# rostin79s/TFHE-AES

Measured on AMD Instinct MI355X. Metric: AES-128 CTR blocks/sec (FHE), higher is better.
Workload: dtype u64+f64; 1 GPU; configs[2]: 128 CTR blocks per GPU, Server::aes_encrypt 10 rounds (1280 bit-CBS/block), counters pre-incremented client-side; params=PARAM_OPT, blocks_per_gpu=128, total_blocks=128

## Files before the change

### include/fheaes.h

```cpp
#ifndef FHEAES_H
#define FHEAES_H

#include <stddef.h>
#include <stdint.h>

#ifdef __cplusplus
extern "C" {
#endif

#define FHEAES_OK 0
#define FHEAES_ERR_INVALID -1
#define FHEAES_ERR_NOKEYS -2
#define FHEAES_ERR_DEVICE -3
#define FHEAES_ERR_NOMEM -4

#define FHEAES_HOST 0
#define FHEAES_DEVICE 1

typedef struct fheaes_params {
    uint32_t lwe_dimension;
    uint32_t glwe_dimension;
    uint32_t polynomial_size;
    uint32_t pbs_base_log;
    uint32_t pbs_level;
// ... 215 lines not shown
int fheaes_profile_reset(fheaes_ctx *ctx);
int fheaes_profile_read(fheaes_ctx *ctx, int stage, double *total_ms, uint64_t *launches, uint64_t *units);

int fheaes_get_twiddles(double *psi_out);
int fheaes_read_bsk_fourier(fheaes_ctx *ctx, uint32_t i, double *out);
int fheaes_k2_launch_plan(uint64_t m, uint32_t cu_count, uint32_t k, int *form, uint64_t *units_main, uint32_t *r_main,
                          uint64_t *units_tail, uint32_t *r_tail);
int fheaes_k2_launch_plan_forms(uint64_t m, uint32_t cu_count, uint32_t k, int allow_pair, int *form, uint64_t *units_main, uint32_t *r_main,
                                uint64_t *units_tail, uint32_t *r_tail);
int fheaes_k2_context_plan(fheaes_ctx *ctx, uint64_t m, int *form, uint64_t *units_main, uint32_t *r_main, uint64_t *units_tail,
                           uint32_t *r_tail, char *kernel, size_t kernel_cap);
int fheaes_k2_set_parking(fheaes_ctx *ctx, int claimed);
int fheaes_k2_set_forms(fheaes_ctx *ctx, int allow_pair, int allow_home);
int fheaes_aes_window_plan(uint64_t n_blocks, uint32_t steps, uint32_t cu_count, uint32_t k, uint64_t *window_blocks, uint64_t *launches,
                           uint64_t *generations, uint64_t *generations_by_round);
int fheaes_aes_context_window(fheaes_ctx *ctx, uint64_t n_blocks, uint32_t steps, uint64_t *window_blocks);
#define FHEAES_AES_WINDOW_OFF 0xFFFFFFFFu
int fheaes_aes_set_window(fheaes_ctx *ctx, uint32_t window_blocks);
#define FHEAES_K2_PARK_SLOTS 1024
int fheaes_k2_park_debug(fheaes_ctx *ctx, const uint32_t *initial_owner, int record);
int fheaes_k2_park_read(fheaes_ctx *ctx, uint64_t *fallbacks, uint64_t *violations, uint32_t *owner_out, uint32_t *record_out,
                        uint64_t record_cap, uint64_t *record_n);
#define FHEAES_WS_BUFFERS 17
#define FHEAES_WS_F64 0
#define FHEAES_WS_WORDS 1
#define FHEAES_WS_TABLES 2
#define FHEAES_WS_PATTERN_F64_HALF 0x7FF87FF8u
#define FHEAES_WS_PATTERN_WORDS 0xA5
#define FHEAES_WS_PATTERN_TABLES 1u
#define FHEAES_WS_POISON_FILL 0
// ... 12 lines not shown
```

### tfhe_aes_amd/_native.py

```python
from __future__ import annotations

import ctypes
import os
import re
from pathlib import Path

import numpy as np

from . import _build
from .params import CParams, WopbsParameters

HOST, DEVICE = 0, 1
MAC_NONE = 0xFFFFFFFF
KW_MIN_SEMIBLOCKS, KW_MAX_SEMIBLOCKS, KW_MAX_KEYS = 2, 8, 4096
AES_WINDOW_OFF = 0xFFFFFFFF
GATE_LWE, GATE_GLWE = 0, 1
K2_PARK_SLOTS = 1024
AUDIT_MAX_ROWS, AUDIT_RECORDS = 256, 16
WS_BUFFERS = 17
WS_CLASSES = ("f64", "words", "tables")
WS_POISON_FILL, WS_POISON_RELEASE = 0, 1
STAGES = ("keyswitch", "blind_rotate", "pfpks", "ggsw_fft", "vertical_packing", "linear")

_u64p = ctypes.POINTER(ctypes.c_uint64)
# ... 111 lines not shown
    "fheaes_gate_plan": (_c.c_int, [_u64p, _c.c_uint64, _c.c_uint32, _u64p, _u32p]),
    "fheaes_profile_enable": (_c.c_int, [_ctx, _c.c_int]),
    "fheaes_profile_reset": (_c.c_int, [_ctx]),
    "fheaes_profile_read": (_c.c_int, [_ctx, _c.c_int, _dp, _u64p, _u64p]),
    "fheaes_get_twiddles": (_c.c_int, [_dp]),
    "fheaes_read_bsk_fourier": (_c.c_int, [_ctx, _c.c_uint32, _dp]),
    "fheaes_k2_launch_plan": (_c.c_int, [_c.c_uint64, _c.c_uint32, _c.c_uint32, _c.POINTER(_c.c_int), _c.POINTER(_c.c_uint64), _c.POINTER(_c.c_uint32),
                                       _c.POINTER(_c.c_uint64), _c.POINTER(_c.c_uint32)]),
    "fheaes_k2_launch_plan_forms": (_c.c_int, [_c.c_uint64, _c.c_uint32, _c.c_uint32, _c.c_int, _c.POINTER(_c.c_int), _c.POINTER(_c.c_uint64),
                                             _c.POINTER(_c.c_uint32), _c.POINTER(_c.c_uint64), _c.POINTER(_c.c_uint32)]),
    "fheaes_k2_context_plan": (_c.c_int, [_ctx, _c.c_uint64, _c.POINTER(_c.c_int), _c.POINTER(_c.c_uint64), _c.POINTER(_c.c_uint32),
                                        _c.POINTER(_c.c_uint64), _c.POINTER(_c.c_uint32), _c.c_char_p, _c.c_size_t]),
    "fheaes_k2_set_parking": (_c.c_int, [_ctx, _c.c_int]),
    "fheaes_k2_set_forms": (_c.c_int, [_ctx, _c.c_int, _c.c_int]),
    "fheaes_aes_window_plan": (_c.c_int, [_c.c_uint64, _c.c_uint32, _c.c_uint32, _c.c_uint32, _u64p, _u64p, _u64p, _u64p]),
    "fheaes_aes_context_window": (_c.c_int, [_ctx, _c.c_uint64, _c.c_uint32, _u64p]),
    "fheaes_aes_set_window": (_c.c_int, [_ctx, _c.c_uint32]),
    "fheaes_k2_park_debug": (_c.c_int, [_ctx, _c.POINTER(_c.c_uint32), _c.c_int]),
    "fheaes_k2_park_read": (_c.c_int, [_ctx, _u64p, _u64p, _c.POINTER(_c.c_uint32), _c.POINTER(_c.c_uint32), _c.c_uint64, _u64p]),
    "fheaes_audit_set": (_c.c_int, [_ctx, _c.c_uint32, _c.c_uint64, _c.c_uint64]),
    "fheaes_audit_rows": (_c.c_int, [_c.c_uint64, _c.c_uint64, _c.c_uint64, _c.c_uint32, _u64p]),
    "fheaes_audit_read": (_c.c_int, [_ctx, _u64p, _u64p, _u64p, _u64p, _c.c_uint64, _u64p]),
    "fheaes_audit_debug": (_c.c_int, [_ctx, _c.c_uint64, _c.c_uint32, _c.c_uint64]),
    "fheaes_workspace_info": (_c.c_int, [_ctx, _c.c_uint32, _c.c_char_p, _c.c_size_t, _u64p, _c.POINTER(_c.c_int), _u64p, _u64p]),
    "fheaes_workspace_poison": (_c.c_int, [_ctx, _c.c_int, _u64p]),
    "fheaes_alloc_debug": (_c.c_int, [_ctx, _c.c_uint64, _u64p]),
    "fheaes_version": (_c.c_char_p, []),
}

_libs = {}
# ... 658 lines not shown
    out = np.zeros(14, dtype=np.uint64)
    rc = load_library().fheaes_aes_public_plan(cnt.ctypes.data_as(_u64p), len(cnt), key_bits, out.ctypes.data_as(_u64p))
    if rc != 0:
        raise FheAesError(rc, "fheaes_aes_public_plan: key_bits must be 128, 192 or 256")
    return [int(x) for x in out[:{128: 10, 192: 12, 256: 14}[key_bits]]]


def aes_window_plan(n_blocks: int, steps: int, cu_count: int = 256, k: int = 4) -> dict:
    w, la, g, gr = _c.c_uint64(), _c.c_uint64(), _c.c_uint64(), _c.c_uint64()
    rc = load_library().fheaes_aes_window_plan(n_blocks, steps, cu_count, k, _c.byref(w), _c.byref(la), _c.byref(g), _c.byref(gr))
    if rc != 0:
        raise FheAesError(rc, "fheaes_aes_window_plan: n_blocks, steps and cu_count must be at least 1")
    return {"window": w.value, "launches": la.value, "generations": g.value, "generations_by_round": gr.value}


def get_twiddles() -> np.ndarray:
    out = np.empty((512, 2), dtype=np.float64)
    rc = load_library().fheaes_get_twiddles(out.ctypes.data_as(_dp))
    if rc != 0:
        raise FheAesError(rc, "fheaes_get_twiddles")
    return out


def gen_lut(nb_block: int, f_table) -> np.ndarray:
    f = np.ascontiguousarray(f_table, dtype=np.uint64)
    if f.size != 1 << nb_block:
        raise ValueError("f_table must have 2^nb_block entries")
    out = np.empty((nb_block, max(512, 1 << nb_block)), dtype=np.uint64)
    rc = load_library().fheaes_gen_lut(nb_block, f.ctypes.data_as(_u64p), out.ctypes.data_as(_u64p))
    if rc != 0:
# ... 3 lines not shown
```

### tfhe_aes_amd/csrc/aes_schedule.h

```cpp
#pragma once

static int many_sbox_dev(fheaes_ctx *c, const uint64_t *bytes, uint64_t n_bytes, int set, uint64_t *out)
{
    return wopbs_dev(c, bytes, n_bytes, 8, c->lutset_d[set], (uint32_t)c->lutset_n[set], 0, out);
}

static int aes_rounds(uint32_t key_bits) { return key_bits == 128 ? 10 : key_bits == 192 ? 12 : key_bits == 256 ? 14 : 0; }

static int check_key_bits(fheaes_ctx *c, uint32_t key_bits)
{
    if (!aes_rounds(key_bits)) return c->fail(FHEAES_ERR_INVALID, "key_bits must be 128, 192 or 256, got %u", key_bits);
    return FHEAES_OK;
}

struct AesStep { int set; uint32_t n_luts; GatherTable table; int key_round; };
struct AesSchedule {
    int first_key_round = 0;
    uint32_t max_luts = 0;
    std::vector<AesStep> steps;
    void add(int set, uint32_t n_luts, const GatherTable &t, int key_round) { steps.push_back({set, n_luts, t, key_round}); max_luts = std::max(max_luts, n_luts); }
};

static AesSchedule aes_encrypt_schedule(int nr)
{
// ... 31 lines not shown
    auto key_of = [&](const AesStep &st, uint64_t first_block) {
        if (st.key_round < 0) return KeySets{nullptr, nullptr, 0};
        return rk.round((uint64_t)st.key_round, sw, first_block);
    };
    const uint64_t w = aes_context_window(c, n_blocks, steps);
    TRY(ensure(c, c->ws_vp, (w ? w : n_blocks) * 16 * sch.max_luts * bw * 8));
    uint64_t *vp = (uint64_t *)c->ws_vp.p;
    TRY(launch_add_bcast(c, state, rk.round((uint64_t)sch.first_key_round, sw), sw, n_blocks));
    if (w == 0) {
        for (const AesStep &st : sch.steps) {
            TRY(many_sbox_dev(c, state, 16 * n_blocks, st.set, vp));
            TRY(launch_gather(c, vp, st.n_luts, key_of(st, 0), state, n_blocks, st.table));
        }
        return FHEAES_OK;
    }
    const uint64_t ggsw_words = (uint64_t)c->k1 * c->k1 * FHE_N, total = steps * n_blocks;
    TRY(ensure_wopbs_ws(c, w * AES_BLOCK_BITS));
    uint64_t *small = (uint64_t *)c->ws_small.p;
    const double2 *ggswf = (const double2 *)c->ws_ggswf.p;
    struct Segment { const AesStep *st; uint64_t first, blocks, row; uint64_t *vp; };
    for (uint64_t i0 = 0; i0 < total; i0 += w) {
        const uint64_t len = std::min<uint64_t>(w, total - i0), s = i0 / n_blocks, b0 = i0 % n_blocks, m = len * AES_BLOCK_BITS;
        Segment seg[2] = {{&sch.steps[s], b0, std::min<uint64_t>(len, n_blocks - b0), 0, vp}, {}};
        int n_seg = 1;
        if (seg[0].blocks < len) {
            seg[1] = {&sch.steps[s + 1], 0, len - seg[0].blocks, seg[0].blocks, vp + seg[0].blocks * 16 * seg[0].st->n_luts * bw};
            n_seg = 2;
        }
        for (int g = 0; g < n_seg; ++g)
            TRY(launch_keyswitch(c, state + seg[g].first * sw, seg[g].blocks * AES_BLOCK_BITS, small + seg[g].row * AES_BLOCK_BITS * (c->n + 1)));
        TRY(cbs_from_small(c, m));
        if (n_seg == 1 || seg[0].st->set == seg[1].st->set) {
            const int set = seg[0].st->set;
            TRY(launch_vertical_packing(c, ggswf, 16 * len, 8, c->lutset_d[set], (uint32_t)c->lutset_n[set], 0, vp));
        } else {
            for (int g = 0; g < n_seg; ++g) {
                const int set = seg[g].st->set;
                TRY(launch_vertical_packing(c, ggswf + seg[g].row * AES_BLOCK_BITS * (ggsw_words / 2), 16 * seg[g].blocks, 8, c->lutset_d[set],
                                            (uint32_t)c->lutset_n[set], 0, seg[g].vp));
            }
        }
        for (int g = 0; g < n_seg; ++g)
            TRY(launch_gather(c, seg[g].vp, seg[g].st->n_luts, key_of(*seg[g].st, seg[g].first), state + seg[g].first * sw, seg[g].blocks, seg[g].st->table));
    }
    return FHEAES_OK;
}

static int aes_encrypt_dev(fheaes_ctx *c, const KeySets &rk, uint64_t *state, uint64_t n_blocks, int nr) { return aes_run_dev(c, rk, state, n_blocks, aes_encrypt_schedule(nr)); }
static int aes_decrypt_dev(fheaes_ctx *c, const KeySets &rk, uint64_t *state, uint64_t n_blocks, int nr) { return aes_run_dev(c, rk, state, n_blocks, aes_decrypt_schedule(nr)); }
static int aes_decrypt_eq_dev(fheaes_ctx *c, const KeySets &dw, uint64_t *state, uint64_t n_blocks, int nr) { return aes_run_dev(c, dw, state, n_blocks, aes_decrypt_eq_schedule(nr)); }

typedef int (*AesDevFn)(fheaes_ctx *, const KeySets &, uint64_t *, uint64_t, int);

static int dec_round_keys_dev(fheaes_ctx *c, const uint64_t *w, uint64_t *dw, int nr, uint64_t n_keys)
// ... 500 lines not shown
```

### tfhe_aes_amd/csrc/engine.hip

```cpp
#include <hip/hip_runtime.h>
#include <algorithm>
#include <cmath>
#include <cstdarg>
#include <cstdio>
#include <atomic>
#include <chrono>
#include <cstring>
#include <functional>
#include <mutex>
#include <string>
#include <type_traits>
#include <unordered_map>
#include <vector>

#include "knobs.h"
#include "fheaes.h"
#include "fft_dev.h"
#include "kern_extprod.h"
#include "kern_gate.h"
#include "kern_blindrot_latency.h"
#include "kern_blindrot16.h"
#include "kern_blindrot_pair.h"
#include "kern_audit.h"
#include "ks_launch.h"
// ... 69 lines not shown
    if (!ctx) return FHEAES_ERR_INVALID;
    CtxLock lock__(ctx);
    if ((allow_pair != 0 && allow_pair != 1) || (allow_home != 0 && allow_home != 1))
        return ctx->fail(FHEAES_ERR_INVALID, "k2_set_forms: each of allow_pair, allow_home is 0 or 1 (got %d, %d)", allow_pair, allow_home);
    HIP_TRY(ctx, hipStreamSynchronize(ctx->stream));
    ctx->k2_deny_pair = allow_pair == 0;
    ctx->k2_deny_home = allow_home == 0;
    return FHEAES_OK;
}
int fheaes_aes_window_plan(uint64_t n_blocks, uint32_t steps, uint32_t cu_count, uint32_t k, uint64_t *window_blocks, uint64_t *launches,
                           uint64_t *generations, uint64_t *generations_by_round)
{
    if (!window_blocks || !launches || !generations || !generations_by_round || n_blocks == 0 || steps == 0 || cu_count == 0) return FHEAES_ERR_INVALID;
    const AesWindowPlan pl = aes_window_plan(n_blocks, steps, cu_count, k + 1);
    *window_blocks = pl.window; *launches = pl.launches; *generations = pl.generations; *generations_by_round = pl.generations_by_round;
    return FHEAES_OK;
}
int fheaes_aes_context_window(fheaes_ctx *ctx, uint64_t n_blocks, uint32_t steps, uint64_t *window_blocks)
{
    if (!ctx) return FHEAES_ERR_INVALID;
    CtxLock lock__(ctx);
    if (!window_blocks) return ctx->fail(FHEAES_ERR_INVALID, "aes_context_window: null output");
    *window_blocks = aes_context_window(ctx, n_blocks, steps);
    return FHEAES_OK;
}
int fheaes_aes_set_window(fheaes_ctx *ctx, uint32_t window_blocks)
{
    if (!ctx) return FHEAES_ERR_INVALID;
    CtxLock lock__(ctx);
    HIP_TRY(ctx, hipStreamSynchronize(ctx->stream));
// ... 1872 lines not shown
```

### tfhe_aes_amd/csrc/engine_launch.h

```cpp
#pragma once

#define MAX_CHUNK_BITS 32768ull
#define K2_CALL_MAX_BITS 65536ull
#define MAX_WOPBS_BITS 16u

namespace {

#define LATENCY_BATCH_BITS 256ull
#define K2_PAIR_MIN_BITS 768ull
struct K2Plan { int form; uint64_t units_main; uint32_t r_main; uint64_t units_tail; uint32_t r_tail; };
K2Plan k2_plan(uint64_t m, uint32_t cu_count, uint32_t k1, bool allow_pair = true)
{
    K2Plan pl{};
    if (m <= LATENCY_BATCH_BITS) { pl.form = 0; pl.units_main = m; pl.r_main = 1; return pl; }
    if (allow_pair && k1 == 5 && m > K2_PAIR_MIN_BITS) {
        pl.form = 2; pl.r_main = 6; pl.r_tail = 4;
        const uint64_t gens = (m + 6ull * cu_count - 1) / (6ull * cu_count);
        uint64_t nu = gens * cu_count;
        uint64_t four = 6 * nu >= m ? (6 * nu - m) / 2 : 0;
        if (four > nu) four = nu;
        if (four == nu && 4 * nu > m) { nu = (m + 3) / 4; four = nu; }
        pl.units_tail = four; pl.units_main = nu - four;
        return pl;
    }
// ... 47 lines not shown
    const uint64_t gen_bits = 6ull * cu_count;
    if (k2_plan(std::min<uint64_t>(n * AES_BLOCK_BITS, MAX_CHUNK_BITS), cu_count, k1, allow_pair).form != 2) return pl;
    if (n * AES_BLOCK_BITS % gen_bits == 0) return pl;
    uint64_t g = AES_BLOCK_BITS, r = gen_bits;
    while (r) { const uint64_t t = g % r; g = r; r = t; }
    const uint64_t base = gen_bits / g;
    const uint64_t w = std::min<uint64_t>(n, AES_WINDOW_MAX_BLOCKS) / base * base;
    if (w == 0) return pl;
    uint64_t launches, generations;
    aes_window_count(n, steps, w, cu_count, k1, &launches, &generations);
    if (generations >= pl.generations_by_round) return pl;
    pl.window = w; pl.launches = launches; pl.generations = generations;
    return pl;
}

int launch_keyswitch(fheaes_ctx *c, const uint64_t *in, uint64_t m, uint64_t *out)
{
    if (m == 0) return FHEAES_OK;
    StageScope sc(c, FHEAES_STAGE_KEYSWITCH, m);
    const uint64_t ct_tiles16 = ((m + KS_CT_TILE - 1) / KS_CT_TILE) * (KS_CT_TILE / 16);
    TRY(ensure(c, c->ws_digits, ct_tiles16 * c->ks_ksteps * 1024));
    int8_t *af = (int8_t *)c->ws_digits.p;
    const uint64_t threads = ct_tiles16 * c->ks_ksteps * 64;
    ks_launch_digits_k1(dim3((unsigned)((threads + 255) / 256)), c->stream, in, (uint64_t)c->big1, c->big, m, c->ks_ksteps, af);
    KeyswitchArgs a{};
    a.afrag = af; a.bfrag = c->ksk_frag; a.ksteps = c->ks_ksteps; a.coltiles = c->ks_coltiles;
    a.in = in; a.in_stride = c->big1; a.body_index = (int32_t)c->big; a.body_col = c->n; a.ncols = c->n + 1;
    a.out = out; a.out_stride = c->n + 1; a.out_z_stride = 0; a.m = m;
    dim3 grid((c->ks_coltiles + KSL_COL_TILES - 1) / KSL_COL_TILES, (unsigned)((m + 16 * KSL_CT_TILES - 1) / (16 * KSL_CT_TILES)), 1);
    ks_launch_mfma_lds(1, grid, c->stream, a);
    HIP_TRY(c, hipGetLastError());
    return FHEAES_OK;
}

int launch_pfpks(fheaes_ctx *c, const uint64_t *in, uint64_t m, uint64_t *out, uint64_t out_stride, int block = -1)
{
    if (m == 0) return FHEAES_OK;
    StageScope sc(c, FHEAES_STAGE_PFPKS, m);
    const uint32_t gsz = c->k1 * FHE_N;
    const uint64_t ct_tiles16 = ((m + KS_CT_TILE - 1) / KS_CT_TILE) * (KS_CT_TILE / 16);
    TRY(ensure(c, c->ws_digits, ct_tiles16 * c->pf_ksteps * 2 * 1024));
    int8_t *af = (int8_t *)c->ws_digits.p;
    const uint64_t threads = ct_tiles16 * c->pf_ksteps * 64;
    ks_launch_digits_k3(dim3((unsigned)((threads + 255) / 256)), c->stream, in, (uint64_t)c->big1, c->big1, m, c->pf_ksteps, af);
    KeyswitchArgs a{};
    a.afrag = af; a.bfrag = c->pfpksk_frag; a.ksteps = c->pf_ksteps; a.coltiles = c->pf_coltiles;
    if (block >= 0) a.bfrag += (size_t)block * c->pf_ksteps * c->pf_coltiles * 8 * 1024;
    a.in = in; a.in_stride = c->big1; a.body_index = -1; a.body_col = 0; a.ncols = gsz;
    a.out = out; a.out_stride = out_stride; a.out_z_stride = block >= 0 ? 0 : gsz; a.m = m;
    dim3 grid((c->pf_coltiles + KSL_COL_TILES - 1) / KSL_COL_TILES, (unsigned)((m + 16 * KSL_CT_TILES - 1) / (16 * KSL_CT_TILES)), block >= 0 ? 1 : c->k1);
    ks_launch_mfma_lds(2, grid, c->stream, a);
    HIP_TRY(c, hipGetLastError());
    return FHEAES_OK;
}

int launch_forward_fourier(fheaes_ctx *c, const uint64_t *in, uint64_t polys, double2 *out, int stage)
{
    if (polys == 0) return FHEAES_OK;
    StageScope sc(c, stage, polys);
    uint64_t wgs = (polys + EP_GROUPS - 1) / EP_GROUPS;
    if (wgs > 8192) wgs = 8192;
    hipLaunchKernelGGL(forward_fourier_kernel, dim3((unsigned)wgs), dim3(EP_THREADS), 0, c->stream, in, out, polys, c->tw_d);
    HIP_TRY(c, hipGetLastError());
    return FHEAES_OK;
}

bool k2_pair_allowed(fheaes_ctx *c)
{
    if (c->k2_deny_pair) return false;
    if (c->k2_pair_ok < 0) {
        int per_cu = 0;
        const hipError_t oe = hipOccupancyMaxActiveBlocksPerMultiprocessor(&per_cu, blind_rotate_pair_kernel<5, 5, 8, 3, 2>, BRP_THREADS, 0);
        c->k2_pair_ok = (oe == hipSuccess && per_cu >= 1) ? 1 : 0;
        (void)hipGetLastError();
    }
    return c->k2_pair_ok == 1;
}
// ... 131 lines not shown
#ifdef EP_STAMPS
    static const char *namesL[EP_NPH] = {"barrier (result) + accumulate", "rotate+decompose (1 coeff x K1)", "read digits + forward fft", "digit stores", "barrier (digits)", "MAC", "barrier (MAC done)",
                                         "products store + next rows", "barrier (products)", "inverse fft -> doubles", "barrier (acc)", "barrier (decomposition)"};
    static const char *namesT[EP_NPH] = {"stage+rotate+decomp_first", "decomp_next", "fwd head", "pre-level barrier", "fwd tail (transpose+dft16)",
                                         "digit stores+late loads", "exchange barrier", "MAC", "products exchange", "inverse fft", "convert+add", "loop head"};
    StampReport rep(c, (size_t)L.grid * (L.threads / 64), L.pl.form == 0 ? namesL : namesT, L.pl.form == 0 ? 8 : 0);
    a.stamps = rep.d;
#endif
    hipLaunchKernelGGL(L.kernel, dim3(L.grid), dim3(L.threads), 0, c->stream, a);
    HIP_TRY(c, hipGetLastError());
    if (c->audit_rows && m >= c->audit_min_bits) TRY(launch_audit(c, a));
    return FHEAES_OK;
}

int launch_vertical_packing(fheaes_ctx *c, const double2 *ggswf, uint64_t n_inputs, uint32_t bits, const uint64_t *luts,
                            uint32_t n_luts, int per_input, uint64_t *out)
{
    if (n_inputs == 0) return FHEAES_OK;
    StageScope sc(c, FHEAES_STAGE_VERTICAL_PACKING, n_inputs * n_luts * bits);
    const bool k4 = c->k1 == 5;
    const uint32_t R = k4 ? 3 : 8;
    void (*const cmux_kernel)(CmuxArgs) = k4 ? cmux_level_kernel<5, 15, 3> : cmux_level_kernel<2, 15, 8>;
    void (*const vp_kernel)(VpArgs) = k4 ? vertical_packing_kernel<5, 15, 3> : vertical_packing_kernel<2, 15, 8>;
    const uint32_t inst_per_input = n_luts * bits;
    const uint64_t W = lut_row_words(bits);
    const uint64_t *glwe_root = nullptr;
    if (bits > 9) {
        const uint32_t tree_bits = bits - 9;
        const uint64_t instances = n_inputs * inst_per_input, gsz = (uint64_t)c->k1 * FHE_N;
        const uint64_t half_words = instances * (1ull << (tree_bits - 1)) * gsz;
        TRY(ensure(c, c->ws_tree, 2 * half_words * 8));
        uint64_t *buf[2] = {(uint64_t *)c->ws_tree.p, (uint64_t *)c->ws_tree.p + half_words};
        for (uint32_t t = 0; t < tree_bits; ++t) {
            CmuxArgs a{};
            a.ggsw = ggswf; a.tw = c->tw_d;
            a.luts = t == 0 ? luts : nullptr; a.in = t == 0 ? nullptr : buf[(t - 1) & 1]; a.out = buf[t & 1];
            a.bits = bits; a.bit = 9 + t; a.nodes_out = 1u << (tree_bits - 1 - t);
            a.inst_per_input = inst_per_input; a.lut_per_input = per_input ? 1 : 0; a.lut_words = W;
            const uint64_t jobs = (uint64_t)inst_per_input * a.nodes_out;
            a.wg_per_input = (uint32_t)((jobs + R - 1) / R);
            hipLaunchKernelGGL(cmux_kernel, dim3((unsigned)(n_inputs * a.wg_per_input)), dim3(EP_THREADS), 0, c->stream, a);
            HIP_TRY(c, hipGetLastError());
        }
        glwe_root = buf[(tree_bits - 1) & 1];
    }
    VpArgs a{};
    a.ggsw = ggswf; a.tw = c->tw_d;
    a.out = out; a.iters = bits < 9 ? bits : 9; a.ggsw_per_input = bits;
    a.luts = luts; a.lut_words = W; a.glwe_in = glwe_root;
    a.lut_per_input = per_input ? 1 : 0; a.inst_per_input = inst_per_input;
    a.wg_per_input = (inst_per_input + R - 1) / R;
    hipLaunchKernelGGL(vp_kernel, dim3((unsigned)(n_inputs * a.wg_per_input)), dim3(EP_THREADS), 0, c->stream, a);
    HIP_TRY(c, hipGetLastError());
    return FHEAES_OK;
}

#define GATE_MAX_GRID 65536ull
uint32_t gate_r(uint32_t k1) { return k1 == 5 ? 3 : 8; }

uint64_t gate_table(const uint64_t *bits_of_gate, uint64_t n_gates, uint32_t R, uint64_t chunk, std::vector<GateWg> *wgs, std::vector<uint64_t> *chunk_end,
                    uint64_t *n_wgs)
{
    uint64_t first = 0, count = 0;
// ... 285 lines not shown
    if (!c) return FHEAES_ERR_INVALID;
    if (!c->have_keys) return c->fail(FHEAES_ERR_NOKEYS, "evaluation keys have not been uploaded");
    return FHEAES_OK;
}

int ensure_wopbs_ws(fheaes_ctx *c, uint64_t bits)
{
    const uint64_t ggsw_words = (uint64_t)c->k1 * c->k1 * FHE_N;
    TRY(ensure(c, c->ws_small, bits * (c->n + 1) * 8));
    TRY(ensure(c, c->ws_pbs, bits * c->big1 * 8));
    TRY(ensure(c, c->ws_ggsw, bits * ggsw_words * 8));
    TRY(ensure(c, c->ws_ggswf, bits * ggsw_words * 8));
    return FHEAES_OK;
}

int cbs_from_small(fheaes_ctx *c, uint64_t m)
{
    const uint64_t ggsw_words = (uint64_t)c->k1 * c->k1 * FHE_N;
    TRY(launch_cbs_pbs(c, (const uint64_t *)c->ws_small.p, m, 1, (uint64_t *)c->ws_pbs.p));
    TRY(launch_pfpks(c, (const uint64_t *)c->ws_pbs.p, m, (uint64_t *)c->ws_ggsw.p, ggsw_words));
    TRY(launch_forward_fourier(c, (const uint64_t *)c->ws_ggsw.p, m * c->k1 * c->k1, (double2 *)c->ws_ggswf.p, FHEAES_STAGE_GGSW_FFT));
    return FHEAES_OK;
}

int cbs_bits(fheaes_ctx *c, const uint64_t *in, uint64_t m)
{
    TRY(launch_keyswitch(c, in, m, (uint64_t *)c->ws_small.p));
    return cbs_from_small(c, m);
}

int wopbs_dev(fheaes_ctx *c, const uint64_t *lwe_in, uint64_t n_inputs, uint32_t bits, const uint64_t *luts, uint32_t n_luts,
              int per_input, uint64_t *lwe_out)
{
    if (bits < 1 || bits > MAX_WOPBS_BITS) return c->fail(FHEAES_ERR_INVALID, "bits_per_input must be in 1..%u (got %u)", MAX_WOPBS_BITS, bits);
    if (n_luts < 1) return c->fail(FHEAES_ERR_INVALID, "n_luts must be >= 1");
    if (n_inputs == 0) return FHEAES_OK;
    uint64_t chunk_inputs = std::max<uint64_t>(1, MAX_CHUNK_BITS / bits);
    if (bits > 9) {
        const uint64_t per_input = (uint64_t)n_luts * bits * (1ull << (bits - 9)) * c->k1 * FHE_N * 8;
        chunk_inputs = std::max<uint64_t>(1, std::min<uint64_t>(chunk_inputs, (2ull << 30) / per_input));
    }
    const uint64_t W = lut_row_words(bits);
    TRY(ensure_wopbs_ws(c, std::min<uint64_t>(n_inputs, chunk_inputs) * bits));
    for (uint64_t i0 = 0; i0 < n_inputs; i0 += chunk_inputs) {
        const uint64_t ni = std::min<uint64_t>(chunk_inputs, n_inputs - i0);
        TRY(cbs_bits(c, lwe_in + i0 * bits * c->big1, ni * bits));
        const uint64_t *l = per_input ? luts + i0 * n_luts * bits * W : luts;
        TRY(launch_vertical_packing(c, (const double2 *)c->ws_ggswf.p, ni, bits, l, n_luts, per_input, lwe_out + i0 * n_luts * bits * c->big1));
    }
    return FHEAES_OK;
}

}
```

### tfhe_aes_amd/csrc/kern_extprod.h

```cpp
#pragma once
#include "fft_dev.h"

#define EP_THREADS 256
#define EP_EARLY_LOAD 2
#define EP_MAC_PRIO 1
#define EP_ROT_CHUNK 4
#define EP_PREFETCH 2
#define EP_MIN_WAVES 2
#define EP_GROUPS 16
#define EP_LDS_DOUBLES (EP_GROUPS * GROUP_TILE_DOUBLES + 2 * FHE_TW_ENTRIES)

__device__ __forceinline__ void ep_load_table(double2 *tw_lds, const double2 *tw_g)
{
    for (int i = threadIdx.x; i < FHE_TW_ENTRIES; i += blockDim.x) tw_lds[i] = tw_g[i];
}

struct ExtProdArgs {
    const double2 *ggsw;
    const double2 *tw;
    uint64_t *out;
    uint64_t count;
    uint32_t iters;
    const uint64_t *lwe_in;
    uint64_t tv_const;
// ... 67 lines not shown
        double2 v = *reinterpret_cast<const double2 *>(tile + 2 * (b + 16 * k2));
        xr[k2] = v.x; xi[k2] = v.y;
    }
    wave_lds_sync();
    nega_inv(xr, xi, tw, tile, b);
}

#ifdef EP_STAMPS
#define EP_NPH 12
#define EP_STAMP(ph) do { unsigned long long t__ = __builtin_readcyclecounter(); ph_cyc[ph] += t__ - t_last; t_last = t__; } while (0)
#else
#define EP_STAMP(ph) do { } while (0)
#endif

struct VpArgs {
    const double2 *ggsw;
    const double2 *tw;
    uint64_t *out;
    uint32_t iters;
    const uint64_t *luts;
    uint32_t lut_per_input;
    uint32_t inst_per_input;
    uint32_t wg_per_input;
    uint32_t ggsw_per_input;
    uint64_t lut_words;
    const uint64_t *glwe_in;
};

template <int K1, int BASE_LOG, int R>
__global__ __launch_bounds__(EP_THREADS, EP_MIN_WAVES) void vertical_packing_kernel(const VpArgs A)
{
    static_assert(R * K1 <= EP_GROUPS, "too many polynomials for 16 lane groups");
    __shared__ __attribute__((aligned(16))) double lds[EP_LDS_DOUBLES];
    double2 *tw = reinterpret_cast<double2 *>(lds + EP_GROUPS * GROUP_TILE_DOUBLES);

    const int tid = threadIdx.x;
    const int g = tid >> 4, b = tid & 15;
    const bool owner = g < R * K1;
    const int r_own = owner ? g / K1 : R - 1;
// ... 14 lines not shown
#pragma unroll
        for (int a = 0; a < 16; ++a) { lo[a] = src[16 * a + b]; hi[a] = src[256 + 16 * a + b]; }
    } else {
        const uint64_t set = A.lut_per_input ? input : 0;
        const uint64_t *lut = A.luts + (set * A.inst_per_input + inst % A.inst_per_input) * A.lut_words;
#pragma unroll
        for (int a = 0; a < 16; ++a) {
            lo[a] = (p_own == K1 - 1) ? lut[16 * a + b] : 0;
            hi[a] = (p_own == K1 - 1) ? lut[256 + 16 * a + b] : 0;
        }
    }
    __syncthreads();

    const size_t ggsw_stride = (size_t)K1 * K1 * FHE_H;

    for (uint32_t it = 0; it < A.iters; ++it) {
        const int t = (1024 - (1 << it)) & 1023;
        const double2 *G = A.ggsw + ((size_t)input * A.ggsw_per_input + it) * ggsw_stride;

        uint64_t *stage = reinterpret_cast<uint64_t *>(tile);
#pragma unroll
        for (int a = 0; a < 16; ++a) {
            stage[16 * a + b] = lo[a];
            stage[256 + 16 * a + b] = hi[a];
        }
        wave_lds_sync();
        double xr[16], xi[16];
#pragma unroll
        for (int a = 0; a < 16; ++a) {
            int j0 = 16 * a + b, j1 = j0 + 256;
            int s0 = (j0 - t) & 511, s1 = (j1 - t) & 511;
            uint64_t v0 = stage[s0], v1 = stage[s1];
            if (((s0 + t) >> 9) & 1) v0 = (uint64_t)0 - v0;
// ... 20 lines not shown
            }
            nega_fwd_tail(xr, xi, tile, b);
            const double2 *Gl = G + tid;
            constexpr int PF = (K1 < EP_PREFETCH) ? K1 : EP_PREFETCH;
            constexpr int EARLY = (EP_EARLY_LOAD < PF) ? EP_EARLY_LOAD : PF;
            constexpr int CHUNK = (K1 * 2 * 2 + 3) / 4;
            double2 bq[PF][K1];
#pragma unroll
            for (int e = 0; e < EARLY; ++e) {
#pragma unroll
                for (int k2 = e * CHUNK; k2 < (e + 1) * CHUNK && k2 < 16; ++k2) {
                    double2 v; v.x = xr[k2]; v.y = xi[k2];
                    *reinterpret_cast<double2 *>(tile + 2 * (b + 16 * k2)) = v;
                }
                __builtin_amdgcn_sched_barrier(0);
#pragma unroll
                for (int c = 0; c < K1; ++c) bq[e][c] = Gl[(size_t)(e * K1 + c) * FHE_H];
                __builtin_amdgcn_sched_barrier(0);
            }
#pragma unroll
            for (int k2 = (EARLY * CHUNK < 16 ? EARLY * CHUNK : 16); k2 < 16; ++k2) {
                double2 v; v.x = xr[k2]; v.y = xi[k2];
                *reinterpret_cast<double2 *>(tile + 2 * (b + 16 * k2)) = v;
            }
            __builtin_amdgcn_sched_barrier(0);
            wg_barrier_lds_only();
            __builtin_amdgcn_s_setprio(EP_MAC_PRIO);
            __builtin_amdgcn_sched_barrier(0);
#pragma unroll
            for (int p = EARLY; p < PF; ++p)
#pragma unroll
                for (int c = 0; c < K1; ++c) bq[p][c] = Gl[(size_t)(p * K1 + c) * FHE_H];
            __builtin_amdgcn_sched_barrier(0);
#pragma unroll
            for (int p = 0; p < K1; ++p) {
                double2 bv[K1];
#pragma unroll
                for (int c = 0; c < K1; ++c) bv[c] = bq[p % PF][c];
                if (p + PF < K1) {
#pragma unroll
                    for (int c = 0; c < K1; ++c) bq[p % PF][c] = Gl[(size_t)((p + PF) * K1 + c) * FHE_H];
                }
                __builtin_amdgcn_sched_barrier(0);
#pragma unroll
                for (int r = 0; r < R; ++r) {
                    double2 d = *reinterpret_cast<const double2 *>(lds + (r * K1 + p) * GROUP_TILE_DOUBLES + 2 * tid);
#pragma unroll
                    for (int c = 0; c < K1; ++c) {
                        fr[r][c] = __builtin_fma(d.x, bv[c].x, fr[r][c]);
                        fr[r][c] = __builtin_fma(-d.y, bv[c].y, fr[r][c]);
                        fi[r][c] = __builtin_fma(d.x, bv[c].y, fi[r][c]);
                        fi[r][c] = __builtin_fma(d.y, bv[c].x, fi[r][c]);
                    }
                }
                __builtin_amdgcn_sched_barrier(0);
            }
            __builtin_amdgcn_s_setprio(0);
        };
        level_body();

        __syncthreads();
#pragma unroll
        for (int r = 0; r < R; ++r)
#pragma unroll
            for (int c = 0; c < K1; ++c) {
                double2 v; v.x = fr[r][c]; v.y = fi[r][c];
                *reinterpret_cast<double2 *>(lds + (r * K1 + c) * GROUP_TILE_DOUBLES + 2 * tid) = v;
// ... 91 lines not shown
            xi[a] = (double)decompose_first<BASE_LOG, 1>(b1 - a1, st);
        }
    }
    __syncthreads();
    ep_product_once<K1, R>(xr, xi, A.ggsw, (uint32_t)(input * A.bits + A.bit), lds, tw, tile, tid, b);
    if (valid) {
        uint64_t *o = A.out + ((inst * A.nodes_out + node) * K1 + p_own) * FHE_N;
#pragma unroll
        for (int a = 0; a < 16; ++a) {
            o[16 * a + b] = c0lo[a] + torus_from_double(xr[a]);
            o[256 + 16 * a + b] = c0hi[a] + torus_from_double(xi[a]);
        }
    }
}

__global__ __launch_bounds__(EP_THREADS) void forward_fourier_kernel(const uint64_t *in, double2 *out, uint64_t polys, const double2 *tw_g)
{
    __shared__ __attribute__((aligned(16))) double lds[EP_LDS_DOUBLES];
    double2 *tw = reinterpret_cast<double2 *>(lds + EP_GROUPS * GROUP_TILE_DOUBLES);
    const int tid = threadIdx.x, g = tid >> 4, b = tid & 15;
    double *tile = lds + g * GROUP_TILE_DOUBLES;
    ep_load_table(tw, tw_g);
    __syncthreads();
    for (uint64_t base = (uint64_t)blockIdx.x * EP_GROUPS; base < polys; base += (uint64_t)gridDim.x * EP_GROUPS) {
        uint64_t q = base + g;
        bool valid = q < polys;
        if (!valid) q = polys - 1;
        const uint64_t *p = in + q * FHE_N;
        double xr[16], xi[16];
#pragma unroll
        for (int a = 0; a < 16; ++a) {
            xr[a] = double_from_torus(p[16 * a + b]);
            xi[a] = double_from_torus(p[256 + 16 * a + b]);
        }
        nega_fwd(xr, xi, tw, tile, b);
        if (valid) {
            double2 *o = out + q * FHE_H;
#pragma unroll
            for (int k2 = 0; k2 < 16; ++k2) { double2 v; v.x = xr[k2]; v.y = xi[k2]; o[b + 16 * k2] = v; }
        }
    }
}
// ... 1 lines not shown
```

### tfhe_aes_amd/csrc/kern_keyswitch.h

```cpp
#pragma once
#include <hip/hip_runtime.h>
#include <stdint.h>
#include "fft_dev.h"

#define KS_CT_TILE 64
#define KS_KSTEP 64

typedef int ks_int4 __attribute__((ext_vector_type(4)));

struct KeyswitchArgs {
    const int8_t *afrag;
    const int8_t *bfrag;
    uint32_t ksteps, coltiles;
    const uint64_t *in;
    uint64_t in_stride;
    int32_t body_index;
    uint32_t body_col;
    uint32_t ncols;
    uint64_t *out;
    uint64_t out_stride, out_z_stride;
    uint64_t m;
};

#define KSL_CT_TILES 8
#define KSL_THREADS (64 * KSL_CT_TILES)
#define KSL_COL_TILES 4

#ifndef FHEAES_KS_DECLS_ONLY
__global__ __launch_bounds__(256) void keybytes_kernel(const uint64_t *key, uint64_t key_z_stride, uint32_t rows, uint32_t ncols,
                                                       uint32_t ksteps, uint32_t coltiles, int8_t *frag)
{
    const uint64_t gid = (uint64_t)blockIdx.x * blockDim.x + threadIdx.x;
    const uint32_t lane = gid & 63;
    const uint64_t t = gid >> 6;
    const uint32_t C = t % coltiles;
    const uint32_t ks = (uint32_t)(t / coltiles);
    const uint32_t z = blockIdx.y;
// ... 125 lines not shown
            for (int pl = 0; pl < PLANES; ++pl) a[t][pl] = *reinterpret_cast<const ks_int4 *>(base + ((wt * 4 + t) * PLANES + pl) * 1024);
#pragma unroll
        for (int s = 0; s < 8; ++s) {
#pragma unroll
            for (int t = 0; t < 4; ++t) acc[t][s] = __builtin_amdgcn_mfma_i32_16x16x64_i8(a[t][0], b[s], acc[t][s], 0, 0, 0);
            if (PLANES == 2 && s >= 1) {
#pragma unroll
                for (int t = 0; t < 4; ++t) acc[t][s] = __builtin_amdgcn_mfma_i32_16x16x64_i8(a[t][1], b[s - 1], acc[t][s], 0, 0, 0);
            }
        }
    }

    const uint32_t C = C0 + wc;
    const uint32_t col = C * 16 + (lane & 15);
    if (C >= A.coltiles || col >= A.ncols) return;
#pragma unroll
    for (int t = 0; t < 4; ++t)
#pragma unroll
        for (int r = 0; r < 4; ++r) {
            const uint64_t ct = (T0 + wt * 4 + t) * 16 + (uint64_t)(lane >> 4) * 4 + r;
            if (ct >= A.m) continue;
            uint64_t v = 0;
#pragma unroll
            for (int s = 0; s < 8; ++s) v += (uint64_t)(int64_t)acc[t][s][r] << (8 * s);
            v = (uint64_t)0 - v;
            if (A.body_index >= 0 && col == A.body_col) v += A.in[ct * A.in_stride + (uint32_t)A.body_index];
            A.out[ct * A.out_stride + (uint64_t)z * A.out_z_stride + col] = v;
        }
}
#endif
```

Baseline: 60.72 blocks/s.

## Reorder CBS rows so bit-0 inputs keep only body GGSW row

```diff
diff --git a/include/fheaes.h b/include/fheaes.h
--- a/include/fheaes.h
+++ b/include/fheaes.h
@@ -253,6 +253,9 @@
 int fheaes_k2_set_forms(fheaes_ctx *ctx, int allow_pair, int allow_home);
 int fheaes_aes_window_plan(uint64_t n_blocks, uint32_t steps, uint32_t cu_count, uint32_t k, uint64_t *window_blocks, uint64_t *launches,
                            uint64_t *generations, uint64_t *generations_by_round);
+int fheaes_cbs_row_plan(uint64_t n_inputs, uint32_t bits, uint32_t k, uint64_t *rows_full, uint64_t *rows_body_only, uint64_t *k3_tiles_full,
+                        uint64_t *k3_tiles_all, uint64_t *int8_mac);
+int fheaes_cbs_row(uint64_t n_inputs, uint32_t bits, uint64_t input, uint32_t bit, uint64_t *row);
 int fheaes_aes_context_window(fheaes_ctx *ctx, uint64_t n_blocks, uint32_t steps, uint64_t *window_blocks);
 #define FHEAES_AES_WINDOW_OFF 0xFFFFFFFFu
 int fheaes_aes_set_window(fheaes_ctx *ctx, uint32_t window_blocks);
diff --git a/tfhe_aes_amd/_native.py b/tfhe_aes_amd/_native.py
--- a/tfhe_aes_amd/_native.py
+++ b/tfhe_aes_amd/_native.py
@@ -149,6 +149,8 @@
     "fheaes_k2_set_parking": (_c.c_int, [_ctx, _c.c_int]),
     "fheaes_k2_set_forms": (_c.c_int, [_ctx, _c.c_int, _c.c_int]),
     "fheaes_aes_window_plan": (_c.c_int, [_c.c_uint64, _c.c_uint32, _c.c_uint32, _c.c_uint32, _u64p, _u64p, _u64p, _u64p]),
+    "fheaes_cbs_row_plan": (_c.c_int, [_c.c_uint64, _c.c_uint32, _c.c_uint32, _u64p, _u64p, _u64p, _u64p, _u64p]),
+    "fheaes_cbs_row": (_c.c_int, [_c.c_uint64, _c.c_uint32, _c.c_uint64, _c.c_uint32, _u64p]),
     "fheaes_aes_context_window": (_c.c_int, [_ctx, _c.c_uint64, _c.c_uint32, _u64p]),
     "fheaes_aes_set_window": (_c.c_int, [_ctx, _c.c_uint32]),
     "fheaes_k2_park_debug": (_c.c_int, [_ctx, _c.POINTER(_c.c_uint32), _c.c_int]),
@@ -837,6 +839,22 @@
     return {"window": w.value, "launches": la.value, "generations": g.value, "generations_by_round": gr.value}
 
 
+def cbs_row_plan(n_inputs: int, bits: int, k: int = 4) -> dict:
+    out = [_c.c_uint64() for _ in range(5)]
+    rc = load_library().fheaes_cbs_row_plan(n_inputs, bits, k, *[_c.byref(o) for o in out])
+    if rc != 0:
+        raise FheAesError(rc, "fheaes_cbs_row_plan: n_inputs in 1..32768, bits in 1..16, k in 1..4")
+    return dict(zip(("rows_full", "rows_body_only", "k3_tiles_full", "k3_tiles_all", "int8_mac"), (o.value for o in out)))
+
+
+def cbs_row(n_inputs: int, bits: int, input: int, bit: int) -> int:
+    row = _c.c_uint64()
+    rc = load_library().fheaes_cbs_row(n_inputs, bits, input, bit, _c.byref(row))
+    if rc != 0:
+        raise FheAesError(rc, "fheaes_cbs_row: input < n_inputs, bit < bits, bits in 1..16")
+    return row.value
+
+
 def get_twiddles() -> np.ndarray:
     out = np.empty((512, 2), dtype=np.float64)
     rc = load_library().fheaes_get_twiddles(out.ctypes.data_as(_dp))
diff --git a/tfhe_aes_amd/csrc/aes_schedule.h b/tfhe_aes_amd/csrc/aes_schedule.h
--- a/tfhe_aes_amd/csrc/aes_schedule.h
+++ b/tfhe_aes_amd/csrc/aes_schedule.h
@@ -69,7 +69,7 @@
         }
         return FHEAES_OK;
     }
-    const uint64_t ggsw_words = (uint64_t)c->k1 * c->k1 * FHE_N, total = steps * n_blocks;
+    const uint64_t total = steps * n_blocks;
     TRY(ensure_wopbs_ws(c, w * AES_BLOCK_BITS));
     uint64_t *small = (uint64_t *)c->ws_small.p;
     const double2 *ggswf = (const double2 *)c->ws_ggswf.p;
@@ -82,17 +82,21 @@
             seg[1] = {&sch.steps[s + 1], 0, len - seg[0].blocks, seg[0].blocks, vp + seg[0].blocks * 16 * seg[0].st->n_luts * bw};
             n_seg = 2;
         }
-        for (int g = 0; g < n_seg; ++g)
-            TRY(launch_keyswitch(c, state + seg[g].first * sw, seg[g].blocks * AES_BLOCK_BITS, small + seg[g].row * AES_BLOCK_BITS * (c->n + 1)));
-        TRY(cbs_from_small(c, m));
+        CbsBatch batch{16 * len, 8, 0};
+        for (int g = 0; g < n_seg; ++g) {
+            batch.first = 16 * seg[g].row;
+            TRY(launch_keyswitch(c, state + seg[g].first * sw, seg[g].blocks * AES_BLOCK_BITS, small, &batch));
+        }
+        TRY(cbs_from_small(c, m, &batch));
         if (n_seg == 1 || seg[0].st->set == seg[1].st->set) {
             const int set = seg[0].st->set;
-            TRY(launch_vertical_packing(c, ggswf, 16 * len, 8, c->lutset_d[set], (uint32_t)c->lutset_n[set], 0, vp));
+            batch.first = 0;
+            TRY(launch_vertical_packing(c, ggswf, 16 * len, 8, c->lutset_d[set], (uint32_t)c->lutset_n[set], 0, vp, &batch));
         } else {
             for (int g = 0; g < n_seg; ++g) {
                 const int set = seg[g].st->set;
-                TRY(launch_vertical_packing(c, ggswf + seg[g].row * AES_BLOCK_BITS * (ggsw_words / 2), 16 * seg[g].blocks, 8, c->lutset_d[set],
-                                            (uint32_t)c->lutset_n[set], 0, seg[g].vp));
+                batch.first = 16 * seg[g].row;
+                TRY(launch_vertical_packing(c, ggswf, 16 * seg[g].blocks, 8, c->lutset_d[set], (uint32_t)c->lutset_n[set], 0, seg[g].vp, &batch));
             }
         }
         for (int g = 0; g < n_seg; ++g)
diff --git a/tfhe_aes_amd/csrc/engine.hip b/tfhe_aes_amd/csrc/engine.hip
--- a/tfhe_aes_amd/csrc/engine.hip
+++ b/tfhe_aes_amd/csrc/engine.hip
@@ -107,6 +107,23 @@
     if (!window_blocks || !launches || !generations || !generations_by_round || n_blocks == 0 || steps == 0 || cu_count == 0) return FHEAES_ERR_INVALID;
     const AesWindowPlan pl = aes_window_plan(n_blocks, steps, cu_count, k + 1);
     *window_blocks = pl.window; *launches = pl.launches; *generations = pl.generations; *generations_by_round = pl.generations_by_round;
+    return FHEAES_OK;
+}
+int fheaes_cbs_row_plan(uint64_t n_inputs, uint32_t bits, uint32_t k, uint64_t *rows_full, uint64_t *rows_body_only, uint64_t *k3_tiles_full,
+                        uint64_t *k3_tiles_all, uint64_t *int8_mac)
+{
+    if (!rows_full || !rows_body_only || !k3_tiles_full || !k3_tiles_all || !int8_mac || n_inputs == 0 || n_inputs > MAX_CHUNK_BITS || bits < 1 ||
+        bits > MAX_WOPBS_BITS || k < 1 || k > 4)
+        return FHEAES_ERR_INVALID;
+    const CbsRowPlan pl = cbs_row_plan(n_inputs, bits, k);
+    *rows_full = pl.rows_full; *rows_body_only = pl.rows_body_only; *k3_tiles_full = pl.k3_tiles_full; *k3_tiles_all = pl.k3_tiles_all;
+    *int8_mac = pl.int8_mac;
+    return FHEAES_OK;
+}
+int fheaes_cbs_row(uint64_t n_inputs, uint32_t bits, uint64_t input, uint32_t bit, uint64_t *row)
+{
+    if (!row || bits < 1 || bits > MAX_WOPBS_BITS || input >= n_inputs || bit >= bits) return FHEAES_ERR_INVALID;
+    *row = cbs_row_plan(n_inputs, bits, 1).rows_body_only ? ks_cbs_row(input, bit, bits, n_inputs) : input * bits + bit;
     return FHEAES_OK;
 }
 int fheaes_aes_context_window(fheaes_ctx *ctx, uint64_t n_blocks, uint32_t steps, uint64_t *window_blocks)
diff --git a/tfhe_aes_amd/csrc/engine_launch.h b/tfhe_aes_amd/csrc/engine_launch.h
--- a/tfhe_aes_amd/csrc/engine_launch.h
+++ b/tfhe_aes_amd/csrc/engine_launch.h
@@ -85,7 +85,21 @@
     return pl;
 }
 
-int launch_keyswitch(fheaes_ctx *c, const uint64_t *in, uint64_t m, uint64_t *out)
+#define K3_TILE_ROWS (16ull * KSL_CT_TILES)
+struct CbsRowPlan { uint64_t rows_full, rows_body_only, k3_tiles_full, k3_tiles_all, int8_mac; };
+CbsRowPlan cbs_row_plan(uint64_t n_inputs, uint32_t bits, uint32_t k)
+{
+    CbsRowPlan pl{};
+    pl.rows_body_only = bits <= 9 ? n_inputs : 0;
+    pl.rows_full = n_inputs * bits - pl.rows_body_only;
+    pl.k3_tiles_full = (pl.rows_full + K3_TILE_ROWS - 1) / K3_TILE_ROWS;
+    pl.k3_tiles_all = (n_inputs * bits + K3_TILE_ROWS - 1) / K3_TILE_ROWS;
+    pl.int8_mac = (pl.rows_full * (k + 1) + pl.rows_body_only) * (((uint64_t)k * FHE_N + 1) * 3) * ((uint64_t)(k + 1) * FHE_N) * 15;
+    return pl;
+}
+struct CbsBatch { uint64_t n_inputs; uint32_t bits; uint64_t first; };
+
+int launch_keyswitch(fheaes_ctx *c, const uint64_t *in, uint64_t m, uint64_t *out, const CbsBatch *batch = nullptr)
 {
     if (m == 0) return FHEAES_OK;
     StageScope sc(c, FHEAES_STAGE_KEYSWITCH, m);
@@ -98,13 +112,18 @@
     a.afrag = af; a.bfrag = c->ksk_frag; a.ksteps = c->ks_ksteps; a.coltiles = c->ks_coltiles;
     a.in = in; a.in_stride = c->big1; a.body_index = (int32_t)c->big; a.body_col = c->n; a.ncols = c->n + 1;
     a.out = out; a.out_stride = c->n + 1; a.out_z_stride = 0; a.m = m;
+    if (batch && batch->bits > 1) {
+        a.out = out + ks_cbs_row(batch->first, 1, batch->bits, batch->n_inputs) * a.out_stride;
+        a.map_bits = batch->bits;
+        a.map_bit0_row = (uint32_t)(ks_cbs_row(batch->first, 0, batch->bits, batch->n_inputs) - ks_cbs_row(batch->first, 1, batch->bits, batch->n_inputs));
+    }
     dim3 grid((c->ks_coltiles + KSL_COL_TILES - 1) / KSL_COL_TILES, (unsigned)((m + 16 * KSL_CT_TILES - 1) / (16 * KSL_CT_TILES)), 1);
     ks_launch_mfma_lds(1, grid, c->stream, a);
     HIP_TRY(c, hipGetLastError());
     return FHEAES_OK;
 }
 
-int launch_pfpks(fheaes_ctx *c, const uint64_t *in, uint64_t m, uint64_t *out, uint64_t out_stride, int block = -1)
+int launch_pfpks(fheaes_ctx *c, const uint64_t *in, uint64_t m, uint64_t *out, uint64_t out_stride, int block = -1, const CbsRowPlan *plan = nullptr)
 {
     if (m == 0) return FHEAES_OK;
     StageScope sc(c, FHEAES_STAGE_PFPKS, m);
@@ -120,18 +139,35 @@
     a.in = in; a.in_stride = c->big1; a.body_index = -1; a.body_col = 0; a.ncols = gsz;
     a.out = out; a.out_stride = out_stride; a.out_z_stride = block >= 0 ? 0 : gsz; a.m = m;
     dim3 grid((c->pf_coltiles + KSL_COL_TILES - 1) / KSL_COL_TILES, (unsigned)((m + 16 * KSL_CT_TILES - 1) / (16 * KSL_CT_TILES)), block >= 0 ? 1 : c->k1);
+    if (block < 0 && plan && plan->rows_body_only) {
+        KeyswitchArgs body = a;
+        body.bfrag += (size_t)c->k * c->pf_ksteps * c->pf_coltiles * 8 * 1024;
+        body.out = out + (uint64_t)c->k * gsz; body.out_z_stride = 0;
+        ks_launch_mfma_lds(2, dim3(grid.x, (unsigned)plan->k3_tiles_all, 1), c->stream, body);
+        if (plan->k3_tiles_full) {
+            a.m = std::min<uint64_t>(m, plan->k3_tiles_full * K3_TILE_ROWS);
+            ks_launch_mfma_lds(2, dim3(grid.x, (unsigned)plan->k3_tiles_full, c->k), c->stream, a);
+        }
+        HIP_TRY(c, hipGetLastError());
+        return FHEAES_OK;
+    }
     ks_launch_mfma_lds(2, grid, c->stream, a);
     HIP_TRY(c, hipGetLastError());
     return FHEAES_OK;
 }
 
-int launch_forward_fourier(fheaes_ctx *c, const uint64_t *in, uint64_t polys, double2 *out, int stage)
-{
-    if (polys == 0) return FHEAES_OK;
-    StageScope sc(c, stage, polys);
-    uint64_t wgs = (polys + EP_GROUPS - 1) / EP_GROUPS;
-    if (wgs > 8192) wgs = 8192;
-    hipLaunchKernelGGL(forward_fourier_kernel, dim3((unsigned)wgs), dim3(EP_THREADS), 0, c->stream, in, out, polys, c->tw_d);
+int launch_forward_fourier(fheaes_ctx *c, const uint64_t *in, uint64_t polys, double2 *out, int stage, uint64_t tail_runs = 0, uint32_t per = 0,
+                           uint32_t stride = 0)
+{
+    if (polys == 0 && tail_runs == 0) return FHEAES_OK;
+    StageScope sc(c, stage, polys + tail_runs * stride);
+    auto launch = [&](const uint64_t *src, double2 *dst, uint64_t n, uint32_t per_, uint32_t stride_) {
+        if (n == 0) return;
+        const uint64_t wgs = std::min<uint64_t>((n + EP_GROUPS - 1) / EP_GROUPS, 8192);
+        hipLaunchKernelGGL(forward_fourier_kernel, dim3((unsigned)wgs), dim3(EP_THREADS), 0, c->stream, src, dst, n, c->tw_d, per_, stride_);
+    };
+    launch(in, out, polys, 0, 0);
+    launch(in + polys * FHE_N, out + polys * FHE_H, tail_runs * per, per, stride);
     HIP_TRY(c, hipGetLastError());
     return FHEAES_OK;
 }
@@ -293,7 +329,7 @@
 }
 
 int launch_vertical_packing(fheaes_ctx *c, const double2 *ggswf, uint64_t n_inputs, uint32_t bits, const uint64_t *luts,
-                            uint32_t n_luts, int per_input, uint64_t *out)
+                            uint32_t n_luts, int per_input, uint64_t *out, const CbsBatch *batch = nullptr)
 {
     if (n_inputs == 0) return FHEAES_OK;
     StageScope sc(c, FHEAES_STAGE_VERTICAL_PACKING, n_inputs * n_luts * bits);
@@ -324,8 +360,15 @@
         glwe_root = buf[(tree_bits - 1) & 1];
     }
     VpArgs a{};
-    a.ggsw = ggswf; a.tw = c->tw_d;
-    a.out = out; a.iters = bits < 9 ? bits : 9; a.ggsw_per_input = bits;
+    const uint64_t gs = (uint64_t)c->k1 * c->k1 * FHE_H;
+    if (batch && bits <= 9) {
+        a.ggsw1 = ggswf + (bits - 1) * batch->first * gs; a.stride1 = (bits - 1) * gs;
+        a.ggsw0 = ggswf + ((bits - 1) * batch->n_inputs + batch->first) * gs; a.stride0 = gs;
+    } else {
+        a.ggsw0 = ggswf; a.ggsw1 = ggswf + gs; a.stride0 = a.stride1 = bits * gs;
+    }
+    a.tw = c->tw_d;
+    a.out = out; a.iters = bits < 9 ? bits : 9;
     a.luts = luts; a.lut_words = W; a.glwe_in = glwe_root;
     a.lut_per_input = per_input ? 1 : 0; a.inst_per_input = inst_per_input;
     a.wg_per_input = (inst_per_input + R - 1) / R;
@@ -641,12 +684,16 @@
     return FHEAES_OK;
 }
 
-int cbs_from_small(fheaes_ctx *c, uint64_t m)
+int cbs_from_small(fheaes_ctx *c, uint64_t m, const CbsBatch *batch = nullptr)
 {
     const uint64_t ggsw_words = (uint64_t)c->k1 * c->k1 * FHE_N;
+    CbsRowPlan pl{};
+    pl.rows_full = m;
+    if (batch) pl = cbs_row_plan(batch->n_inputs, batch->bits, c->k);
     TRY(launch_cbs_pbs(c, (const uint64_t *)c->ws_small.p, m, 1, (uint64_t *)c->ws_pbs.p));
-    TRY(launch_pfpks(c, (const uint64_t *)c->ws_pbs.p, m, (uint64_t *)c->ws_ggsw.p, ggsw_words));
-    TRY(launch_forward_fourier(c, (const uint64_t *)c->ws_ggsw.p, m * c->k1 * c->k1, (double2 *)c->ws_ggswf.p, FHEAES_STAGE_GGSW_FFT));
+    TRY(launch_pfpks(c, (const uint64_t *)c->ws_pbs.p, m, (uint64_t *)c->ws_ggsw.p, ggsw_words, -1, batch ? &pl : nullptr));
+    TRY(launch_forward_fourier(c, (const uint64_t *)c->ws_ggsw.p, pl.rows_full * c->k1 * c->k1, (double2 *)c->ws_ggswf.p, FHEAES_STAGE_GGSW_FFT,
+                               pl.rows_body_only, c->k1, c->k1 * c->k1));
     return FHEAES_OK;
 }
 
@@ -671,11 +718,13 @@
     TRY(ensure_wopbs_ws(c, std::min<uint64_t>(n_inputs, chunk_inputs) * bits));
     for (uint64_t i0 = 0; i0 < n_inputs; i0 += chunk_inputs) {
         const uint64_t ni = std::min<uint64_t>(chunk_inputs, n_inputs - i0);
-        TRY(cbs_bits(c, lwe_in + i0 * bits * c->big1, ni * bits));
+        const CbsBatch batch_rows{ni, bits, 0}, *const batch = cbs_row_plan(ni, bits, c->k).rows_body_only ? &batch_rows : nullptr;
+        TRY(launch_keyswitch(c, lwe_in + i0 * bits * c->big1, ni * bits, (uint64_t *)c->ws_small.p, batch));
+        TRY(cbs_from_small(c, ni * bits, batch));
         const uint64_t *l = per_input ? luts + i0 * n_luts * bits * W : luts;
-        TRY(launch_vertical_packing(c, (const double2 *)c->ws_ggswf.p, ni, bits, l, n_luts, per_input, lwe_out + i0 * n_luts * bits * c->big1));
-    }
-    return FHEAES_OK;
-}
-
-}
+        TRY(launch_vertical_packing(c, (const double2 *)c->ws_ggswf.p, ni, bits, l, n_luts, per_input, lwe_out + i0 * n_luts * bits * c->big1, batch));
+    }
+    return FHEAES_OK;
+}
+
+}
diff --git a/tfhe_aes_amd/csrc/kern_extprod.h b/tfhe_aes_amd/csrc/kern_extprod.h
--- a/tfhe_aes_amd/csrc/kern_extprod.h
+++ b/tfhe_aes_amd/csrc/kern_extprod.h
@@ -105,7 +105,8 @@
 #endif
 
 struct VpArgs {
-    const double2 *ggsw;
+    const double2 *ggsw0, *ggsw1;
+    uint64_t stride0, stride1;
     const double2 *tw;
     uint64_t *out;
     uint32_t iters;
@@ -113,7 +114,6 @@
     uint32_t lut_per_input;
     uint32_t inst_per_input;
     uint32_t wg_per_input;
-    uint32_t ggsw_per_input;
     uint64_t lut_words;
     const uint64_t *glwe_in;
 };
@@ -158,9 +158,13 @@
 
     const size_t ggsw_stride = (size_t)K1 * K1 * FHE_H;
 
-    for (uint32_t it = 0; it < A.iters; ++it) {
+    const uint32_t lut_iters = (A.glwe_in || A.iters == 0) ? 0 : 1;
+#pragma unroll
+    for (int phase = 0; phase < 2; ++phase)
+    for (uint32_t it = phase ? lut_iters : 0; it < (phase ? A.iters : lut_iters); ++it) {
         const int t = (1024 - (1 << it)) & 1023;
-        const double2 *G = A.ggsw + ((size_t)input * A.ggsw_per_input + it) * ggsw_stride;
+        const double2 *G = it ? A.ggsw1 + (size_t)input * A.stride1 + (size_t)(it - 1) * ggsw_stride : A.ggsw0 + (size_t)input * A.stride0;
+        const int p_first = phase == 0 ? K1 - 1 : 0;
 
         uint64_t *stage = reinterpret_cast<uint64_t *>(tile);
 #pragma unroll
@@ -211,8 +215,10 @@
                     *reinterpret_cast<double2 *>(tile + 2 * (b + 16 * k2)) = v;
                 }
                 __builtin_amdgcn_sched_barrier(0);
-#pragma unroll
-                for (int c = 0; c < K1; ++c) bq[e][c] = Gl[(size_t)(e * K1 + c) * FHE_H];
+                if (e >= p_first) {
+#pragma unroll
+                    for (int c = 0; c < K1; ++c) bq[e][c] = Gl[(size_t)(e * K1 + c) * FHE_H];
+                }
                 __builtin_amdgcn_sched_barrier(0);
             }
 #pragma unroll
@@ -226,28 +232,34 @@
             __builtin_amdgcn_sched_barrier(0);
 #pragma unroll
             for (int p = EARLY; p < PF; ++p)
-#pragma unroll
-                for (int c = 0; c < K1; ++c) bq[p][c] = Gl[(size_t)(p * K1 + c) * FHE_H];
+                if (p >= p_first) {
+#pragma unroll
+                    for (int c = 0; c < K1; ++c) bq[p][c] = Gl[(size_t)(p * K1 + c) * FHE_H];
+                }
             __builtin_amdgcn_sched_barrier(0);
 #pragma unroll
             for (int p = 0; p < K1; ++p) {
                 double2 bv[K1];
-#pragma unroll
-                for (int c = 0; c < K1; ++c) bv[c] = bq[p % PF][c];
-                if (p + PF < K1) {
+                if (p >= p_first) {
+#pragma unroll
+                    for (int c = 0; c < K1; ++c) bv[c] = bq[p % PF][c];
+                }
+                if (p + PF < K1 && p + PF >= p_first) {
 #pragma unroll
                     for (int c = 0; c < K1; ++c) bq[p % PF][c] = Gl[(size_t)((p + PF) * K1 + c) * FHE_H];
                 }
                 __builtin_amdgcn_sched_barrier(0);
-#pragma unroll
-                for (int r = 0; r < R; ++r) {
-                    double2 d = *reinterpret_cast<const double2 *>(lds + (r * K1 + p) * GROUP_TILE_DOUBLES + 2 * tid);
-#pragma unroll
-                    for (int c = 0; c < K1; ++c) {
-                        fr[r][c] = __builtin_fma(d.x, bv[c].x, fr[r][c]);
-                        fr[r][c] = __builtin_fma(-d.y, bv[c].y, fr[r][c]);
-                        fi[r][c] = __builtin_fma(d.x, bv[c].y, fi[r][c]);
-                        fi[r][c] = __builtin_fma(d.y, bv[c].x, fi[r][c]);
+                if (p >= p_first) {
+#pragma unroll
+                    for (int r = 0; r < R; ++r) {
+                        double2 d = *reinterpret_cast<const double2 *>(lds + (r * K1 + p) * GROUP_TILE_DOUBLES + 2 * tid);
+#pragma unroll
+                        for (int c = 0; c < K1; ++c) {
+                            fr[r][c] = __builtin_fma(d.x, bv[c].x, fr[r][c]);
+                            fr[r][c] = __builtin_fma(-d.y, bv[c].y, fr[r][c]);
+                            fi[r][c] = __builtin_fma(d.x, bv[c].y, fi[r][c]);
+                            fi[r][c] = __builtin_fma(d.y, bv[c].x, fi[r][c]);
+                        }
                     }
                 }
                 __builtin_amdgcn_sched_barrier(0);
@@ -369,7 +381,8 @@
     }
 }
 
-__global__ __launch_bounds__(EP_THREADS) void forward_fourier_kernel(const uint64_t *in, double2 *out, uint64_t polys, const double2 *tw_g)
+__global__ __launch_bounds__(EP_THREADS) void forward_fourier_kernel(const uint64_t *in, double2 *out, uint64_t polys, const double2 *tw_g,
+                                                                     uint32_t per, uint32_t stride)
 {
     __shared__ __attribute__((aligned(16))) double lds[EP_LDS_DOUBLES];
     double2 *tw = reinterpret_cast<double2 *>(lds + EP_GROUPS * GROUP_TILE_DOUBLES);
@@ -381,6 +394,7 @@
         uint64_t q = base + g;
         bool valid = q < polys;
         if (!valid) q = polys - 1;
+        if (per) q = q / per * stride + (stride - per) + q % per;
         const uint64_t *p = in + q * FHE_N;
         double xr[16], xi[16];
 #pragma unroll
diff --git a/tfhe_aes_amd/csrc/kern_keyswitch.h b/tfhe_aes_amd/csrc/kern_keyswitch.h
--- a/tfhe_aes_amd/csrc/kern_keyswitch.h
+++ b/tfhe_aes_amd/csrc/kern_keyswitch.h
@@ -17,10 +17,17 @@
     int32_t body_index;
     uint32_t body_col;
     uint32_t ncols;
+    uint32_t map_bits : 4, map_bit0_row : 28;
     uint64_t *out;
     uint64_t out_stride, out_z_stride;
     uint64_t m;
 };
+static_assert(sizeof(KeyswitchArgs) == 88, "K3's launches must keep the argument block they were measured with");
+
+__host__ __device__ inline uint64_t ks_cbs_row(uint64_t input, uint32_t bit, uint32_t bits, uint64_t n_inputs)
+{
+    return bit ? (uint64_t)(bits - 1) * input + bit - 1 : (uint64_t)(bits - 1) * n_inputs + input;
+}
 
 #define KSL_CT_TILES 8
 #define KSL_THREADS (64 * KSL_CT_TILES)
@@ -176,6 +183,7 @@
     const uint32_t C = C0 + wc;
     const uint32_t col = C * 16 + (lane & 15);
     if (C >= A.coltiles || col >= A.ncols) return;
+    const uint32_t map_bits = PLANES == 1 ? A.map_bits : 0, map_inv = map_bits ? 0xFFFFFFFFu / map_bits + 1 : 0;
 #pragma unroll
     for (int t = 0; t < 4; ++t)
 #pragma unroll
@@ -187,7 +195,12 @@
             for (int s = 0; s < 8; ++s) v += (uint64_t)(int64_t)acc[t][s][r] << (8 * s);
             v = (uint64_t)0 - v;
             if (A.body_index >= 0 && col == A.body_col) v += A.in[ct * A.in_stride + (uint32_t)A.body_index];
-            A.out[ct * A.out_stride + (uint64_t)z * A.out_z_stride + col] = v;
+            uint64_t row = ct;
+            if (PLANES == 1 && map_bits) {
+                const uint32_t input = __umulhi((uint32_t)ct, map_inv), bit = (uint32_t)ct - input * map_bits;
+                row = bit ? ks_cbs_row(input, bit, map_bits, 0) : A.map_bit0_row + input;
+            }
+            A.out[row * A.out_stride + (uint64_t)z * A.out_z_stride + col] = v;
         }
 }
 #endif
```

Result: no change. 61.17 blocks/s (median of 6 runs) (+0.7%).
